# rbarile17/kelpie

Measured on AMD Instinct MI355X. Metric: candidate explanations evaluated/sec (incl. post-train) + rank-delta match rate, higher is better.
Workload: dtype bf16x3 (fp32-emulated)

## Files before the change

### kelpie_amd/csrc/kp_attn3.hpp

```cpp
#pragma once
#include <type_traits>

#include "kp_attn.hpp"

#ifdef KP_ATTN3_STAMPS
#ifndef KP_DIAGNOSTIC_BUILD
#error "KP_ATTN3_STAMPS is a diagnostic build (make diag / tools/attn_micro.sh)"
#endif
__device__ unsigned long long g_attn3_stamps[8];
#define KP3_STAMP(v) v = __builtin_amdgcn_s_memtime()
#define KP3_ACC(i, a, b) st_acc[i] += (b) - (a)
#else
#define KP3_STAMP(v) (void)0
#define KP3_ACC(i, a, b) (void)0
#endif

#ifdef KP_ATTN3_CLOCK
#ifndef KP_DIAGNOSTIC_BUILD
#error "KP_ATTN3_CLOCK is a diagnostic build (tools/attn_micro.sh)"
#endif
__device__ unsigned long long g_attn3_clock[4096][4];
#endif

#ifndef KP_O_AHEAD
#define KP_O_AHEAD 1
#endif
#ifndef KP_S_AHEAD
#define KP_S_AHEAD 1
#endif
static_assert(KP_S_AHEAD >= 1 && KP_S_AHEAD <= 2, "KP_S_AHEAD: 1..2 (lgkmcnt holds at most 15)");
#if (defined(KP_DIAG_NO_S) || defined(KP_DIAG_NO_O) || defined(KP_ATTN_NODMA) || defined(KP_DIAG_DMA_LGKM0) || \
     defined(KP_DMA_SPREAD_ALL) || defined(KP_DIAG_S4) || defined(KP_DIAG_DMA_VM0) || defined(KP_DIAG_M0SAVE) || defined(KP_DIAG_NO_OSTORE) || defined(KP_DIAG_EARLY_EXIT) || defined(KP_DIAG_O_HALF) || defined(KP_DIAG_S_HALF) || defined(KP_DIAG_XTILE_W)) && \
    !defined(KP_DIAGNOSTIC_BUILD)
#error "kp_attn3 diagnostic define without KP_DIAGNOSTIC_BUILD (these builds compute wrong results: make diag)"
#endif
#ifndef KP_DMA_SPREAD
#define KP_DMA_SPREAD 1
#endif
#ifndef KP_DMA_SPREAD_BCE
#define KP_DMA_SPREAD_BCE 0
#endif
#ifndef KP_ILV
#define KP_ILV 1
#endif
#ifndef KP_DMA_GROUP
#define KP_DMA_GROUP 1
#endif
#ifndef KP_ATTN_PRIO
#define KP_ATTN_PRIO 0
#endif
#ifndef KP_ATTN_FULLTILE
#define KP_ATTN_FULLTILE 1
#endif
#ifndef KP_ATTN_FULLTILE_ALL
#define KP_ATTN_FULLTILE_ALL 0
#endif
#ifndef KP_CV_EXACT_BCE
#define KP_CV_EXACT_BCE 0
#endif
#ifndef KP_ASM_ALL
#define KP_ASM_ALL 0
#endif
#ifndef KP_ASM_MIN_DB
#define KP_ASM_MIN_DB 13
#endif
#ifndef KP_O_NT
#define KP_O_NT 0
#endif
#ifndef KP_O_SC1
#define KP_O_SC1 0
#endif
#ifndef KP_BUF_DMA
#define KP_BUF_DMA 1
#endif
#ifdef KP_DIAG_NO_O
#define KP_DIAG_O false
#else
#define KP_DIAG_O true
#endif
static_assert(KP_O_AHEAD >= 1 && KP_O_AHEAD <= 2, "KP_O_AHEAD: 1..2 (lgkmcnt holds at most 15)");

namespace kpattn {

constexpr float kPosInf = __builtin_huge_valf();

typedef __bf16 bf16x8 __attribute__((ext_vector_type(8)));
typedef __bf16 bf16x4 __attribute__((ext_vector_type(4)));
typedef short s16x4 __attribute__((ext_vector_type(4)));

__host__ __device__ constexpr int split3_row_bytes(int DP) { return 3 * 2 * DP + ((DP / 16) % 2 ? 0 : 32); }
__host__ __device__ constexpr int split3_tile_bytes(int DP) { return 32 * split3_row_bytes(DP); }
__host__ __device__ constexpr int split3_pieces(int DP) { return (split3_tile_bytes(DP) + 1023) / 1024; }
__host__ __device__ constexpr bool attn3_asm(int DB) { return DB >= KP_ASM_MIN_DB || KP_ASM_ALL; }
__host__ __device__ constexpr bool attn3_bufdma(int DB) { return attn3_asm(DB) && KP_ILV && KP_BUF_DMA; }
__host__ __device__ constexpr int attn3_buf_pieces(int DB) {
  return attn3_bufdma(DB) ? (split3_pieces(16 * DB) + 3) / 4 * 4 : split3_pieces(16 * DB);
}
constexpr size_t attn3_lds_bytes(int DB) { return 2u * 1024u * (size_t)attn3_buf_pieces(DB); }

__device__ __forceinline__ void split3(float x, __bf16& h, __bf16& m, __bf16& l) {
  h = (__bf16)x;
  const float r1 = __fsub_rn(x, (float)h);
  m = (__bf16)r1;
  const float r2 = __fsub_rn(r1, (float)m);
  l = (__bf16)r2;
}

typedef __bf16 bf16v4 __attribute__((__vector_size__(8)));
template <bool ASM>
__device__ __forceinline__ bf16x8 lds_rd_bf8(uint32_t addr, int off) {
  if constexpr (ASM) {
    bf16x8 v;
    asm volatile("ds_read_b128 %0, %1 offset:%2" : "=v"(v) : "v"(addr), "i"(off));
    return v;
  } else {
    return *reinterpret_cast<const __attribute__((address_space(3))) bf16x8*>((uintptr_t)(addr + off));
  }
}
template <bool ASM>
__device__ __forceinline__ bf16x4 lds_rd_bf4(uint32_t addr, int off) {
  if constexpr (ASM) {
    bf16x4 v;
    asm volatile("ds_read_b64 %0, %1 offset:%2" : "=v"(v) : "v"(addr), "i"(off));
    return v;
  } else {
    return *reinterpret_cast<const __attribute__((address_space(3))) bf16x4*>((uintptr_t)(addr + off));
  }
}
template <bool ASM>
__device__ __forceinline__ bf16x4 lds_rd_tr(uint32_t addr, int off) {
  if constexpr (ASM) {
    bf16x4 v;
    asm volatile("ds_read_b64_tr_b16 %0, %1 offset:%2" : "=v"(v) : "v"(addr), "i"(off));
    return v;
  } else {
    const bf16v4 v = __builtin_amdgcn_ds_read_tr16_b64_v4bf16(
        reinterpret_cast<__attribute__((address_space(3))) bf16v4*>((uintptr_t)(addr + off)));
    return __builtin_bit_cast(bf16x4, v);
  }
}
template <bool ASM>
__device__ __forceinline__ bf16x8 tied3(bf16x8 v) {
  if constexpr (ASM) asm volatile("" : "+v"(v));
  return v;
}
template <bool ASM>
__device__ __forceinline__ bf16x4 tied3(bf16x4 v) {
  if constexpr (ASM) asm volatile("" : "+v"(v));
  return v;
}
template <bool ASM, int N>
__device__ __forceinline__ void lgkm_wait3() {
  if constexpr (ASM) lgkm_wait<N>();
}

constexpr int kPA[6] = {2, 1, 0, 1, 0, 0};
constexpr int kPB[6] = {0, 1, 2, 0, 1, 0};

__device__ __forceinline__ f32x4 mfma3(const bf16x8 (&a)[3], const bf16x8 (&b)[3], f32x4 c) {
  c = __builtin_amdgcn_mfma_f32_16x16x32_bf16(a[2], b[0], c, 0, 0, 0);
  c = __builtin_amdgcn_mfma_f32_16x16x32_bf16(a[1], b[1], c, 0, 0, 0);
  c = __builtin_amdgcn_mfma_f32_16x16x32_bf16(a[0], b[2], c, 0, 0, 0);
  c = __builtin_amdgcn_mfma_f32_16x16x32_bf16(a[1], b[0], c, 0, 0, 0);
  c = __builtin_amdgcn_mfma_f32_16x16x32_bf16(a[0], b[1], c, 0, 0, 0);
  c = __builtin_amdgcn_mfma_f32_16x16x32_bf16(a[0], b[0], c, 0, 0, 0);
  return c;
}
__device__ __forceinline__ f32x4 mfma3_k16(const bf16x4 (&a)[3], const bf16x4 (&b)[3], f32x4 c) {
#define KP_M16(x, y) \
  c = __builtin_amdgcn_mfma_f32_16x16x16bf16_1k(__builtin_bit_cast(s16x4, x), __builtin_bit_cast(s16x4, y), c, 0, 0, 0)
  KP_M16(a[2], b[0]);
  KP_M16(a[1], b[1]);
  KP_M16(a[0], b[2]);
  KP_M16(a[1], b[0]);
  KP_M16(a[0], b[1]);
  KP_M16(a[0], b[0]);
#undef KP_M16
  return c;
}

template <int DP>
__global__ void kp_split3_table(const float* __restrict__ E, int n_ent, uint8_t* __restrict__ out) {
  const long long i = (long long)blockIdx.x * blockDim.x + threadIdx.x;
  if (i >= (long long)n_ent * (DP / 2)) return;
  const int e = (int)(i / (DP / 2)), d = 2 * (int)(i % (DP / 2));
  __bf16 h[2], m[2], l[2];
  split3(E[(size_t)e * DP + d], h[0], m[0], l[0]);
  split3(E[(size_t)e * DP + d + 1], h[1], m[1], l[1]);
  __bf16* row = reinterpret_cast<__bf16*>(out + (size_t)e * split3_row_bytes(DP));
  row[d] = h[0];
  row[d + 1] = h[1];
  row[DP + d] = m[0];
  row[DP + d + 1] = m[1];
  row[2 * DP + d] = l[0];
  row[2 * DP + d + 1] = l[1];
}

template <int DB, int MODE>
constexpr int attn3_min_wgs() { return (MODE == ATT_BCE_O && 2 * attn3_lds_bytes(DB) <= 163840) ? 2 : 1; }

template <int DB, int MODE>
__global__ __launch_bounds__(256, (attn3_min_wgs<DB, MODE>())) void kp_attn3(const uint8_t* __restrict__ E3, int n_ent,
                                                   const float* __restrict__ Qpre, int nq, AttnWork wk,
                                                   float* __restrict__ out_m, float* __restrict__ out_l,
                                                   float* __restrict__ out_O, const float* __restrict__ qscale,
                                                   float ylo, const double* __restrict__ colpre) {
  constexpr bool WITH_O = MODE != ATT_SOFTMAX;
  constexpr int DP = 16 * DB;
  constexpr bool ASM = attn3_asm(DB);
  constexpr bool ILV = ASM && KP_ILV;
  constexpr int NK = DP / 32;
  constexpr int TAIL = (DP % 32) / 16;
  constexpr int KT = 32;
  constexpr int PART_B = 2 * DP;
  constexpr int ROW_B = split3_row_bytes(DP);
  constexpr bool BUFDMA = attn3_bufdma(DB);
  constexpr int PIECES = attn3_buf_pieces(DB);
  constexpr int BUF_B = 1024 * PIECES;
  extern __shared__ __attribute__((aligned(16))) uint8_t lds3[];

  const int tid = threadIdx.x;
#ifdef KP_DIAG_EARLY_EXIT
  if (ylo != 12345.f) return;
#endif
  if constexpr (KP_ATTN_PRIO > 0) __builtin_amdgcn_s_setprio(KP_ATTN_PRIO);
  const int lane = tid & 63;
  const int w = __builtin_amdgcn_readfirstlane(tid >> 6);
  const int g = lane >> 4, c = lane & 15;
  int key_begin = 0, key_end = 0;
  const uint32_t lds0 = (uint32_t)(uintptr_t)(__attribute__((address_space(3))) uint8_t*)lds3;
#ifdef KP_ATTN3_STAMPS
  unsigned long long st0 = 0, st1 = 0, st2 = 0, st3 = 0, st4 = 0;
  unsigned long long st_acc[5] = {0, 0, 0, 0, 0};
#endif

  const __amdgpu_buffer_rsrc_t e3rsrc = __builtin_amdgcn_make_buffer_rsrc(
      const_cast<uint8_t*>(E3), (short)0, (int)((n_ent + 31) / 32 * 32 * ROW_B + 1024), 0x00020000);
#if KP_O_SC1
  const __amdgpu_buffer_rsrc_t orsrc =
      __builtin_amdgcn_make_buffer_rsrc(out_O, (short)0, 0x7FFFFFFF, 0x00020000);
#endif
  auto bdma = [&](int tile, int buf, int p) {
    __builtin_amdgcn_raw_ptr_buffer_load_lds(
        e3rsrc, (__attribute__((address_space(3))) void*)(uintptr_t)(lds0 + (uint32_t)(buf * BUF_B + 1024 * p)), 16,
        16 * lane, (key_begin + tile * KT) * ROW_B + 1024 * p, 0, 0);
  };
  typedef int i32x4_t __attribute__((ext_vector_type(4)));
  const i32x4_t e3rs = {(int)(uint32_t)(uintptr_t)E3,
                        (int)(uint32_t)((uintptr_t)E3 >> 32) & 0xFFFF,
                        (int)((n_ent + 31) / 32 * 32 * ROW_B + 1024), 0x00020000};
  auto dma_group = [&](int tile, int buf, int g) {
    const int pb = w * ((PIECES + 3) / 4) + 4 * g;
    const uint32_t m0v = (uint32_t)__builtin_amdgcn_readfirstlane((int)(lds0 + (uint32_t)(buf * BUF_B + 1024 * pb)));
    const uint32_t so = (uint32_t)__builtin_amdgcn_readfirstlane((key_begin + tile * KT) * ROW_B + 1024 * pb);
    const int nleft = (PIECES + 3) / 4 - 4 * g;
    uint32_t keep;
    if (nleft >= 4)
      asm volatile(
          "s_mov_b32 %0, m0\n\ts_nop 4\n\ts_mov_b32 m0, %1\n\ts_nop 0\n\t"
          "buffer_load_dwordx4 %2, %3, %4 offen lds\n\t"
          "buffer_load_dwordx4 %2, %3, %4 offen offset:1024 lds\n\t"
          "buffer_load_dwordx4 %2, %3, %4 offen offset:2048 lds\n\t"
          "buffer_load_dwordx4 %2, %3, %4 offen offset:3072 lds\n\ts_mov_b32 m0, %0" : "=&s"(keep) : "s"(m0v),
          "v"(16 * lane), "s"(e3rs), "s"(so)
          : "memory");
    else if (nleft == 3)
      asm volatile(
          "s_mov_b32 %0, m0\n\ts_nop 4\n\ts_mov_b32 m0, %1\n\ts_nop 0\n\t"
          "buffer_load_dwordx4 %2, %3, %4 offen lds\n\t"
          "buffer_load_dwordx4 %2, %3, %4 offen offset:1024 lds\n\t"
          "buffer_load_dwordx4 %2, %3, %4 offen offset:2048 lds\n\ts_mov_b32 m0, %0" : "=&s"(keep) : "s"(m0v),
          "v"(16 * lane), "s"(e3rs), "s"(so)
          : "memory");
    else if (nleft == 2)
      asm volatile(
          "s_mov_b32 %0, m0\n\ts_nop 4\n\ts_mov_b32 m0, %1\n\ts_nop 0\n\t"
          "buffer_load_dwordx4 %2, %3, %4 offen lds\n\t"
          "buffer_load_dwordx4 %2, %3, %4 offen offset:1024 lds\n\ts_mov_b32 m0, %0" : "=&s"(keep) : "s"(m0v),
          "v"(16 * lane), "s"(e3rs), "s"(so)
          : "memory");
    else if (nleft == 1)
      asm volatile(
          "s_mov_b32 %0, m0\n\ts_nop 4\n\ts_mov_b32 m0, %1\n\ts_nop 0\n\t"
          "buffer_load_dwordx4 %2, %3, %4 offen lds\n\ts_mov_b32 m0, %0" : "=&s"(keep) : "s"(m0v),
          "v"(16 * lane), "s"(e3rs), "s"(so)
          : "memory");
  };
  constexpr bool DGROUP = KP_DMA_GROUP && BUFDMA;
  auto issue = [&](int tile, int buf) {
    const uint8_t* src = E3 + (size_t)(key_begin + tile * KT) * ROW_B + 16 * lane;
    if constexpr (KP_DMA_GROUP && BUFDMA) {
#pragma unroll
      for (int g = 0; g < ((PIECES + 3) / 4 + 3) / 4; ++g) dma_group(tile, buf, g);
      return;
    }
#pragma unroll
    for (int p0 = 0; p0 < PIECES; p0 += 4) {
      const int p = p0 + w;
      if constexpr (BUFDMA)
        bdma(tile, buf, p);
      else if (p < PIECES)
        glds16<ASM>(reinterpret_cast<const float*>(src + 1024 * p),
               __builtin_amdgcn_readfirstlane(lds0 + (uint32_t)(buf * BUF_B + 1024 * p)));
    }
  };
  constexpr int NPW = (PIECES + 3) / 4;
  constexpr int SPM = MODE == ATT_BCE_O ? KP_DMA_SPREAD_BCE : KP_DMA_SPREAD;
#ifdef KP_DMA_SPREAD_ALL
  constexpr bool SPREAD = SPM && WITH_O && KP_DIAG_O;
#else
  constexpr bool SPREAD = SPM && ASM && WITH_O && KP_DIAG_O;
#endif
  constexpr int NSLOT = (DP / 32 + (DP % 32) / 16) + (SPM == 3 ? 0 : DB);
  constexpr bool SPREAD2 = SPREAD && ILV && SPM >= 2;
  auto issue_piece = [&](int tile, int buf, int k) {
    const int p = 4 * k + w;
    if constexpr (BUFDMA)
      bdma(tile, buf, p);
    else if (p < PIECES)
      glds16<ASM>(reinterpret_cast<const float*>(E3 + (size_t)(key_begin + tile * KT) * ROW_B + 16 * lane + 1024 * p),
             __builtin_amdgcn_readfirstlane(lds0 + (uint32_t)(buf * BUF_B + 1024 * p)));
  };
  auto dma_slot = [&](int tile, int buf, int slot) {
#pragma unroll
    for (int k = 0; k < NPW; ++k)
      if ((k * NSLOT) / NPW == slot) issue_piece(tile, buf, k);
  };
#ifdef KP_ATTN3_CLOCK
  unsigned long long ck_t0, ck_r0;
  asm volatile("s_memtime %0\n\ts_memrealtime %1\n\ts_waitcnt lgkmcnt(0)" : "=s"(ck_t0), "=s"(ck_r0)::"memory");
#endif
  const int QT = (nq + 63) / 64;
  const long long total = (long long)QT * wk.ktq;
  long long it = wk.ranges ? 0 : (long long)blockIdx.x * wk.per_wg;
  const long long it_end = wk.ranges ? 0 : min(total, it + (long long)wk.per_wg);
  const int n_units = QT * wk.ranges;
  int unit = ((int)gridDim.x % 8 == 0) ? (int)(blockIdx.x % 8) * (int)(gridDim.x / 8) + (int)(blockIdx.x / 8)
                                       : (int)blockIdx.x;
  for (;;) {
    int qt, kt0, kt1, part;
    bool fill_rest;
    if (wk.ranges) {
      if (unit >= n_units) break;
      qt = unit % QT;
      part = unit / QT;
      kt0 = (int)((long long)part * wk.ktq / wk.ranges);
      kt1 = (int)((long long)(part + 1) * wk.ktq / wk.ranges);
      fill_rest = false;
      unit += (int)gridDim.x;
    } else {
      if (it >= it_end) break;
      qt = (int)(it / wk.ktq);
      kt0 = (int)(it - (long long)qt * wk.ktq);
      kt1 = (int)min((long long)wk.ktq, (long long)kt0 + (it_end - it));
      part = (int)blockIdx.x - (int)(((long long)qt * wk.ktq) / wk.per_wg);
      fill_rest = kt1 == wk.ktq;
      it += kt1 - kt0;
    }
    key_begin = kt0 * KT;
    key_end = min(n_ent, kt1 * KT);
    const int ntiles = kt1 - kt0;
    const int q = qt * 64 + 16 * w + c;
    const bool valid = q < nq;
    bf16x8 qb[NK > 0 ? NK : 1][3];
    bf16x4 qt4[3];
    float gsc = 0.f;
    if (MODE == ATT_BCE_O) gsc = valid ? qscale[q] : 0.f;
    {
      const float* qp = Qpre + (size_t)(valid ? q : 0) * DP;
#pragma unroll
      for (int s = 0; s < NK; ++s) {
        const float4 v0 = *reinterpret_cast<const float4*>(qp + 32 * s + 8 * g);
        const float4 v1 = *reinterpret_cast<const float4*>(qp + 32 * s + 8 * g + 4);
        const float f[8] = {v0.x, v0.y, v0.z, v0.w, v1.x, v1.y, v1.z, v1.w};
#pragma unroll
        for (int j = 0; j < 8; ++j) {
          __bf16 h, m, l;
          split3(valid ? f[j] : 0.f, h, m, l);
          qb[s][0][j] = h;
          qb[s][1][j] = m;
          qb[s][2][j] = l;
        }
      }
      if (TAIL) {
        const float4 v0 = *reinterpret_cast<const float4*>(qp + 32 * NK + 4 * g);
        const float f[4] = {v0.x, v0.y, v0.z, v0.w};
#pragma unroll
        for (int j = 0; j < 4; ++j) {
          __bf16 h, m, l;
          split3(valid ? f[j] : 0.f, h, m, l);
          qt4[0][j] = h;
          qt4[1][j] = m;
          qt4[2][j] = l;
        }
      }
    }
    f32x4 O[WITH_O ? DB : 1];
    float m_ref = kNegInf, l_run = 0.f;
    float csh = 0.f;

    for (int pass = 0; pass < 2; ++pass) {
#pragma unroll
      for (int j = 0; j < (WITH_O ? DB : 1); ++j) O[j] = (f32x4){0.f, 0.f, 0.f, 0.f};
      l_run = 0.f;
      float m_seen = kNegInf;
      if (ntiles > 0) issue(0, 0);
      asm volatile("s_waitcnt vmcnt(0)" ::: "memory");
      __syncthreads();
#ifdef KP_DIAG_XTILE_W
      float scp[2][4] = {{0.f, 0.f, 0.f, 0.f}, {0.f, 0.f, 0.f, 0.f}};
      float pwn[8] = {0.f, 0.f, 0.f, 0.f, 0.f, 0.f, 0.f, 0.f};
      float lacc = 0.f;
      bf16x8 pbn[3];
      float dtmp[8], htmp[8];
      auto wpiece = [&](int q) {
        if (q < 24) {
          const int j = q / 3, st = q % 3;
          if (st == 0) {
            dtmp[j] = scp[j >> 2][j & 3] - m_ref;
            m_seen = fmaxf(m_seen, scp[j >> 2][j & 3]);
          } else if (st == 1) {
            pwn[j] = __expf(dtmp[j]);
          } else {
            pwn[j] = __fsub_rn(pwn[j], csh);
            lacc += pwn[j];
          }
        } else if (q < 48) {
          const int j = (q - 24) / 3, st = (q - 24) % 3;
          if (st == 0) {
            const __bf16 h = (__bf16)pwn[j];
            pbn[0][j] = h;
            htmp[j] = __fsub_rn(pwn[j], (float)h);
          } else if (st == 1) {
            const __bf16 m = (__bf16)htmp[j];
            pbn[1][j] = m;
            htmp[j] = __fsub_rn(htmp[j], (float)m);
          } else {
            pbn[2][j] = (__bf16)htmp[j];
          }
        }
      };
#endif

      for (int t = 0; t < ntiles; ++t) {
        const int k0 = key_begin + t * KT;
        KP3_STAMP(st0);
        const bool dma_on = BUFDMA || t + 1 < ntiles;
        const int tn = t + 1 < ntiles ? t + 1 : t;
        const uint32_t tb = lds0 + (uint32_t)((t & 1) * BUF_B);
#if !defined(KP_ATTN_NODMA) && defined(KP_DMA_EARLY)
        if (t + 1 < ntiles) issue(t + 1, (t + 1) & 1);
#endif
        f32x4 sc[2] = {(f32x4){0.f, 0.f, 0.f, 0.f}, (f32x4){0.f, 0.f, 0.f, 0.f}};
#ifdef KP_DIAG_S4
        f32x4 sc4[2] = {(f32x4){0.f, 0.f, 0.f, 0.f}, (f32x4){0.f, 0.f, 0.f, 0.f}};
#endif
        const uint32_t rb = tb + (uint32_t)(c * ROW_B + 16 * g);
        const uint32_t rbt = rb - 8u * g;
        constexpr uint32_t SUB_B = 16u * ROW_B;
        static_assert(SUB_B + 3 * PART_B + 64 * NK < 65536, "LDS read offsets exceed the 16-bit offset field");
        constexpr int SA = ILV ? 2 : KP_S_AHEAD;
        constexpr int LAST = NK + TAIL - 1;
        bf16x8 ra[SA + 1][2][3];
        bf16x4 rt[2][3];
        auto load_full = [&](int s, int b) {
#pragma unroll
          for (int u = 0; u < 2; ++u)
#pragma unroll
            for (int p = 0; p < 3; ++p) ra[b][u][p] = lds_rd_bf8<ASM>(rb, (int)(u * SUB_B) + p * PART_B + 64 * s);
        };
        auto load_tail = [&]() {
#pragma unroll
          for (int u = 0; u < 2; ++u)
#pragma unroll
            for (int p = 0; p < 3; ++p)
              rt[u][p] = lds_rd_bf4<ASM>(rbt, (int)(u * SUB_B) + p * PART_B + 64 * NK);
        };
        auto load_step = [&](int j) {
          if (j < NK)
            load_full(j, j % (SA + 1));
          else
            load_tail();
        };
#ifndef KP_DIAG_NO_S
        if constexpr (ILV) {
          load_step(0);
          if (LAST >= 1) load_step(1);
#pragma unroll
          for (int s = 0; s <= LAST; ++s) {
            if (s < LAST)
              lgkm_wait<6>();
            else
              lgkm_wait<0>();
            __builtin_amdgcn_sched_barrier(0);
#if !defined(KP_ATTN_NODMA)
            if (SPREAD2 && dma_on) {
              dma_slot(tn, (t + 1) & 1, s);
              __builtin_amdgcn_sched_barrier(0);
            }
#endif
            const int b = s % 3;
#pragma unroll
            for (int k = 0; k < 6; ++k) {
#pragma unroll
              for (int u = 0; u < 2; ++u) {
#ifdef KP_DIAG_S4
                f32x4& acc = (s & 1) ? sc4[u] : sc[u];
#else
                f32x4& acc = sc[u];
#endif
                if (s < NK)
                  acc = __builtin_amdgcn_mfma_f32_16x16x32_bf16(ra[b][u][kPA[k]], qb[s < NK ? s : 0][kPB[k]], acc, 0, 0,
                                                               0);
                else
                  acc = __builtin_amdgcn_mfma_f32_16x16x16bf16_1k(__builtin_bit_cast(s16x4, rt[u][kPA[k]]),
                                                                  __builtin_bit_cast(s16x4, qt4[kPB[k]]), acc, 0, 0, 0);
#ifdef KP_DIAG_S_HALF
                if (u == 0 && s + 2 <= LAST && (k & 1) == 0) {
#else
                if (u == 0 && s + 2 <= LAST) {
#endif
                  const int j = s + 2, uu = k & 1, pp = k >> 1;
                  if (j < NK)
                    ra[j % 3][uu][pp] = lds_rd_bf8<true>(rb, (int)(uu * SUB_B) + pp * PART_B + 64 * j);
                  else
                    rt[uu][pp] = lds_rd_bf4<true>(rbt, (int)(uu * SUB_B) + pp * PART_B + 64 * NK);
                }
#ifdef KP_DIAG_XTILE_W
                if (u == 1 && WITH_O) wpiece(6 * s + k);
#endif
                __builtin_amdgcn_sched_barrier(0);
              }
            }
          }
#ifdef KP_DIAG_S4
          sc[0] += sc4[0];
          sc[1] += sc4[1];
#endif
        } else {
#pragma unroll
        for (int j = 0; j < SA && j <= LAST; ++j) load_step(j);
#pragma unroll
        for (int s = 0; s < NK; ++s) {
          if (s + SA <= LAST) {
            load_step(s + SA);
            lgkm_wait3<ASM, 6 * SA>();
          } else if (LAST - s >= 2) {
            lgkm_wait3<ASM, 12>();
          } else if (LAST - s == 1) {
            lgkm_wait3<ASM, 6>();
          } else {
            lgkm_wait3<ASM, 0>();
          }
#pragma unroll
          for (int u = 0; u < 2; ++u) {
            bf16x8 a[3];
#pragma unroll
            for (int p = 0; p < 3; ++p) a[p] = tied3<ASM>(ra[s % (SA + 1)][u][p]);
            sc[u] = mfma3(a, qb[s], sc[u]);
          }
        }
        if (TAIL) {
          lgkm_wait3<ASM, 0>();
#pragma unroll
          for (int u = 0; u < 2; ++u) {
            bf16x4 a[3];
#pragma unroll
            for (int p = 0; p < 3; ++p) a[p] = tied3<ASM>(rt[u][p]);
            sc[u] = mfma3_k16(a, qt4, sc[u]);
          }
        }
        }
#endif
#if !defined(KP_ATTN_NODMA) && !defined(KP_DMA_EARLY)
        if (!SPREAD && t + 1 < ntiles) issue(t + 1, (t + 1) & 1);
#endif
        const uint32_t ob = tb + (uint32_t)((4 * g + (c >> 2)) * ROW_B + 8 * (c & 3));
        constexpr int OA = ILV ? 2 : KP_O_AHEAD;
        bf16x4 ol[OA + 1][3], oh[OA + 1][3];
        auto load_o = [&](int m, int b) {
#pragma unroll
          for (int p = 0; p < 3; ++p) {
            ol[b][p] = lds_rd_tr<ASM>(ob, p * PART_B + 32 * m);
            oh[b][p] = lds_rd_tr<ASM>(ob, 16 * ROW_B + p * PART_B + 32 * m);
          }
        };
        KP3_STAMP(st1);
        if (WITH_O && KP_DIAG_O) {
#pragma unroll
          for (int m = 0; m < OA && m < DB; ++m) load_o(m, m);
        }
        float pw[2][4];
        auto weights = [&](auto full_c) {
          constexpr bool FULL = decltype(full_c)::value;
          auto keep = [&](int u, int r) { return FULL || (k0 + 16 * u + 4 * g + r < key_end); };
        if (MODE == ATT_BCE_O) {
#pragma unroll
          for (int u = 0; u < 2; ++u)
#pragma unroll
            for (int r = 0; r < 4; ++r) {
#if KP_CV_EXACT_BCE & 1
              const float x0 = 1.0f / (1.0f + expf(-sc[u][r]));
#else
              const float x0 = __builtin_amdgcn_rcpf(1.0f + __expf(-sc[u][r]));
#endif
              const float w0 = (1.0f - x0) * x0;
#if KP_CV_EXACT_BCE & 2
              const float gw = w0 >= 1e-12f ? (x0 - ylo) * gsc
                                            : (((x0 - ylo) * __builtin_amdgcn_rcpf(1e-12f)) * gsc) * w0;
              pw[u][r] = keep(u, r) ? gw : 0.f;
#else
              pw[u][r] = keep(u, r) ? (((x0 - ylo) * __builtin_amdgcn_rcpf(fmaxf(w0, 1e-12f))) * gsc) * w0 : 0.f;
#endif
            }
        } else {
          float v[2][4];
          float tmax = kNegInf;
#pragma unroll
          for (int u = 0; u < 2; ++u)
#pragma unroll
            for (int r = 0; r < 4; ++r) {
              v[u][r] = keep(u, r) ? sc[u][r] : kNegInf;
              tmax = fmaxf(tmax, v[u][r]);
            }
          m_seen = fmaxf(m_seen, tmax);
          if (pass == 0 && t == 0) {
            float mq = fmaxf(tmax, __shfl_xor(tmax, 16, 64));
            m_ref = fmaxf(mq, __shfl_xor(mq, 32, 64));
          }
#pragma unroll
          for (int u = 0; u < 2; ++u)
#pragma unroll
            for (int r = 0; r < 4; ++r) pw[u][r] = __expf(v[u][r] - m_ref);
        }
        {
          if (t == 0) {
            float mn = kPosInf;
#pragma unroll
            for (int u = 0; u < 2; ++u)
#pragma unroll
              for (int r = 0; r < 4; ++r)
                if (keep(u, r)) mn = fminf(mn, pw[u][r]);
            mn = fminf(mn, __shfl_xor(mn, 16, 64));
            mn = fminf(mn, __shfl_xor(mn, 32, 64));
            csh = (mn < kPosInf) ? mn : 0.f;
          }
          float lt = 0.f;
#pragma unroll
          for (int u = 0; u < 2; ++u) {
#pragma unroll
            for (int r = 0; r < 4; ++r) pw[u][r] = keep(u, r) ? __fsub_rn(pw[u][r], csh) : 0.f;
            lt += (pw[u][0] + pw[u][1]) + (pw[u][2] + pw[u][3]);
          }
          l_run += lt;
        }
        };
#ifdef KP_DIAG_XTILE_W
        if (t == 0 || !ILV || !WITH_O)
#endif
        if (KP_ATTN_FULLTILE && (ASM || KP_ATTN_FULLTILE_ALL) && k0 + KT <= key_end)
          weights(std::true_type{});
        else
          weights(std::false_type{});
        if (WITH_O && KP_DIAG_O) {
          bf16x8 pb[3];
#ifdef KP_DIAG_XTILE_W
          if (ILV && t > 0) {
            pb[0] = pbn[0];
            pb[1] = pbn[1];
            pb[2] = pbn[2];
            l_run += lacc;
            lacc = 0.f;
          } else
#endif
#pragma unroll
          for (int j = 0; j < 8; ++j) {
            __bf16 h, m, l;
            split3(pw[j >> 2][j & 3], h, m, l);
            pb[0][j] = h;
            pb[1][j] = m;
            pb[2][j] = l;
          }
#ifdef KP_DIAG_XTILE_W
#pragma unroll
          for (int u = 0; u < 2; ++u)
#pragma unroll
            for (int r = 0; r < 4; ++r) scp[u][r] = sc[u][r];
#endif
          KP3_STAMP(st2);
#pragma unroll
          for (int m = 0; m < DB; ++m) {
#if !defined(KP_ATTN_NODMA) && !defined(KP_DMA_EARLY)
            if (DGROUP && SPREAD && !SPREAD2 && dma_on) {
              if (m % 4 == 0 && m < NPW) dma_group(tn, (t + 1) & 1, m / 4);
              if (m == DB - 1)
                for (int g = (DB + 3) / 4; 4 * g < NPW; ++g) dma_group(tn, (t + 1) & 1, g);
            } else if (SPREAD && !SPREAD2 && dma_on) {
              if (m < NPW) {
                issue_piece(tn, (t + 1) & 1, m);
#ifdef KP_DIAG_DMA_LGKM0
                asm volatile("s_waitcnt lgkmcnt(0)" ::: "memory");
#endif
#ifdef KP_DIAG_DMA_VM0
                asm volatile("s_waitcnt vmcnt(0)" ::: "memory");
#endif
              }
              if (m == DB - 1)
                for (int k = DB; k < NPW; ++k) issue_piece(tn, (t + 1) & 1, k);
            }
#endif
            if constexpr (ILV) {
              if (m + 1 < DB)
                lgkm_wait<6>();
              else
                lgkm_wait<0>();
              __builtin_amdgcn_sched_barrier(0);
#if !defined(KP_ATTN_NODMA)
              if (SPREAD2 && dma_on) {
                dma_slot(tn, (t + 1) & 1, NK + TAIL + m);
                __builtin_amdgcn_sched_barrier(0);
              }
#endif
              bf16x8 a[3];
#pragma unroll
              for (int p = 0; p < 3; ++p) {
                const bf16x4 x = ol[m % 3][p], y = oh[m % 3][p];
                a[p] = (bf16x8){x[0], x[1], x[2], x[3], y[0], y[1], y[2], y[3]};
              }
#pragma unroll
              for (int k = 0; k < 6; ++k) {
                O[m] = __builtin_amdgcn_mfma_f32_16x16x32_bf16(a[kPA[k]], pb[kPB[k]], O[m], 0, 0, 0);
#ifdef KP_DIAG_O_HALF
                if (m + 2 < DB && ((m + 2) & 1) == 0) {
#else
                if (m + 2 < DB) {
#endif
                  const int mm = m + 2, pp = k >> 1;
                  if (k & 1)
                    oh[mm % 3][pp] = lds_rd_tr<true>(ob, 16 * ROW_B + pp * PART_B + 32 * mm);
                  else
                    ol[mm % 3][pp] = lds_rd_tr<true>(ob, pp * PART_B + 32 * mm);
                }
                __builtin_amdgcn_sched_barrier(0);
              }
              continue;
            }
            if (m + OA < DB) {
              load_o(m + OA, (m + OA) % (OA + 1));
              lgkm_wait3<ASM, 6 * OA>();
            } else if (DB - 1 - m >= 2) {
              lgkm_wait3<ASM, 12>();
            } else if (DB - 1 - m == 1) {
              lgkm_wait3<ASM, 6>();
            } else {
              lgkm_wait3<ASM, 0>();
            }
            bf16x8 a[3];
#pragma unroll
            for (int p = 0; p < 3; ++p) {
              const bf16x4 x = tied3<ASM>(ol[m % (OA + 1)][p]), y = tied3<ASM>(oh[m % (OA + 1)][p]);
              a[p] = (bf16x8){x[0], x[1], x[2], x[3], y[0], y[1], y[2], y[3]};
            }
            O[m] = mfma3(a, pb, O[m]);
          }
        }
        KP3_STAMP(st3);
        asm volatile("s_waitcnt vmcnt(0)" ::: "memory");
        __syncthreads();
        KP3_STAMP(st4);
        KP3_ACC(0, st0, st1);
        KP3_ACC(1, st1, st2);
        KP3_ACC(2, st2, st3);
        KP3_ACC(3, st3, st4);
#ifdef KP_ATTN3_STAMPS
        st_acc[4] += 1;
#endif
      }
      if (MODE == ATT_BCE_O) break;
      float mq = fmaxf(m_seen, __shfl_xor(m_seen, 16, 64));
      mq = fmaxf(mq, __shfl_xor(mq, 32, 64));
#if defined(KP_DIAG_NO_S) || defined(KP_DIAG_NO_O)
      break;
#endif
      if (pass == 1 || !__syncthreads_or(mq > m_ref + kMargin)) break;
      m_ref = mq;
    }

    float l_tot = l_run + __shfl_xor(l_run, 16, 64);
    l_tot += __shfl_xor(l_tot, 32, 64);
    if (ntiles > 0) {
      l_tot = __fmaf_rn(csh, (float)(key_end - key_begin), l_tot);
      if (WITH_O) {
        const double* p0 = colpre + (size_t)kt0 * DP;
        const double* p1 = colpre + (size_t)kt1 * DP;
#pragma unroll
        for (int m = 0; m < DB; ++m) {
          const int d = 16 * m + 4 * g;
          const double2 a0 = *reinterpret_cast<const double2*>(p0 + d), a1 = *reinterpret_cast<const double2*>(p0 + d + 2);
          const double2 b0 = *reinterpret_cast<const double2*>(p1 + d), b1 = *reinterpret_cast<const double2*>(p1 + d + 2);
          O[m][0] = __fmaf_rn(csh, (float)(b0.x - a0.x), O[m][0]);
          O[m][1] = __fmaf_rn(csh, (float)(b0.y - a0.y), O[m][1]);
          O[m][2] = __fmaf_rn(csh, (float)(b1.x - a1.x), O[m][2]);
          O[m][3] = __fmaf_rn(csh, (float)(b1.y - a1.y), O[m][3]);
        }
      }
    }
    if (valid) {
      const size_t o = (size_t)part * nq + q;
      if (g == 0 && MODE != ATT_BCE_O) {
        out_m[o] = m_ref;
        out_l[o] = l_tot;
      }
#ifdef KP_DIAG_NO_OSTORE
      if (false) {
#else
      if (WITH_O) {
#endif
        float* dst = out_O + o * DP;
#pragma unroll
        for (int m = 0; m < DB; ++m) {
#if KP_O_SC1
          typedef unsigned int u32x4_t __attribute__((ext_vector_type(4)));
          __builtin_amdgcn_raw_buffer_store_b128(__builtin_bit_cast(u32x4_t, O[m]), orsrc,
                                                 (int)((o * DP + 16 * m + 4 * g) * sizeof(float)), 0, 16);
#elif KP_O_NT
          __builtin_nontemporal_store(O[m], reinterpret_cast<f32x4*>(dst + 16 * m + 4 * g));
#else
          *reinterpret_cast<float4*>(dst + 16 * m + 4 * g) = make_float4(O[m][0], O[m][1], O[m][2], O[m][3]);
#endif
        }
      }
    }
    if (fill_rest && valid) {
      for (int pp = part + 1; pp < wk.n_parts; ++pp) {
        const size_t o = (size_t)pp * nq + q;
        if (g == 0 && MODE != ATT_BCE_O) {
          out_m[o] = kNegInf;
          out_l[o] = 0.f;
        }
        if (WITH_O) {
          float* dst = out_O + o * DP;
          for (int d = 4 * g; d < DP; d += 16) *reinterpret_cast<float4*>(dst + d) = make_float4(0.f, 0.f, 0.f, 0.f);
        }
      }
    }
  }
#ifdef KP_ATTN3_STAMPS
  if (lane == 0)
    for (int i = 0; i < 5; ++i) atomicAdd(&g_attn3_stamps[i], st_acc[i]);
#endif
#ifdef KP_ATTN3_CLOCK
  {
    unsigned long long ck_t1, ck_r1;
    asm volatile("s_waitcnt vmcnt(0)\n\ts_memtime %0\n\ts_memrealtime %1\n\ts_waitcnt lgkmcnt(0)"
                 : "=s"(ck_t1), "=s"(ck_r1)::"memory");
    if (tid == 0 && blockIdx.x < 4096) {
      g_attn3_clock[blockIdx.x][0] = ck_t0;
      g_attn3_clock[blockIdx.x][1] = ck_r0;
      g_attn3_clock[blockIdx.x][2] = ck_t1;
      g_attn3_clock[blockIdx.x][3] = ck_r1;
    }
  }
#endif
}

template <int DB>
const uint8_t* split3_image(kp_ctx* c) {
  constexpr int DP = 16 * DB;
  KP_REQUIRE(c->dp == DP, "attn3: table stride mismatch");
  if (!c->e3_ready) {
    const size_t n_pad = (size_t)(c->n_ent + 31) / 32 * 32;
    const size_t bytes = n_pad * split3_row_bytes(DP) + 1024;
    uint8_t* d = reinterpret_cast<uint8_t*>(c->e3.ensure(bytes));
    KP_HIP(hipMemsetAsync(d, 0, bytes, c->stream));
    const long long n = (long long)c->n_ent * (DP / 2);
    hipLaunchKernelGGL((kp_split3_table<DP>), dim3((unsigned)((n + 255) / 256)), dim3(256), 0, c->stream, c->dE,
                       c->n_ent, d);
    KP_HIP(hipGetLastError());
    c->e3_ready = true;
  }
  return c->e3.as<uint8_t>();
}

template <int DP>
__global__ void kp_tile_sums(const float* __restrict__ E, int n_ent, double* __restrict__ ts) {
  const int t = blockIdx.x, d = threadIdx.x;
  if (d >= DP) return;
  double s = 0.0;
  const int e1 = min(n_ent, 32 * t + 32);
  for (int e = 32 * t; e < e1; ++e) s += (double)E[(size_t)e * DP + d];
  ts[(size_t)t * DP + d] = s;
}
template <int DP>
__global__ void kp_tile_prefix(const double* __restrict__ ts, int ntiles, double* __restrict__ pre) {
  const int d = blockIdx.x * blockDim.x + threadIdx.x;
  if (d >= DP) return;
  double s = 0.0;
  pre[d] = 0.0;
  for (int t = 0; t < ntiles; ++t) {
    s += ts[(size_t)t * DP + d];
    pre[(size_t)(t + 1) * DP + d] = s;
  }
}
template <int DB>
const double* tile_prefix(kp_ctx* c) {
  constexpr int DP = 16 * DB;
  if (!c->e3pre_ready) {
    const int ntiles = (c->n_ent + 31) / 32;
    double* ts = reinterpret_cast<double*>(c->e3ts.ensure(sizeof(double) * (size_t)ntiles * DP));
    double* pre = reinterpret_cast<double*>(c->e3pre.ensure(sizeof(double) * (size_t)(ntiles + 1) * DP));
    hipLaunchKernelGGL((kp_tile_sums<DP>), dim3((unsigned)ntiles), dim3((DP + 63) / 64 * 64), 0, c->stream, c->dE,
                       c->n_ent, ts);
    KP_HIP(hipGetLastError());
    hipLaunchKernelGGL((kp_tile_prefix<DP>), dim3((DP + 63) / 64), dim3(64), 0, c->stream, ts, ntiles, pre);
    KP_HIP(hipGetLastError());
    c->e3pre_ready = true;
  }
  return c->e3pre.as<double>();
}

template <int DB, int MODE = ATT_SOFTMAX_O>
int attn3_wpc(kp_ctx* c) {
  static_assert(MODE == ATT_SOFTMAX_O || MODE == ATT_BCE_O, "attn3_wpc: the launched O mode");
  int& slot = c->attn3_wpc[MODE == ATT_BCE_O ? 1 : 0];
  if (slot <= 0) {
    int n = 0;
    KP_HIP(hipOccupancyMaxActiveBlocksPerMultiprocessor(&n, kp_attn3<DB, MODE>, 256, attn3_lds_bytes(DB)));
    slot = std::max(1, n);
  }
  return slot;
}

#define KP_DB_CASE(N, DB_MIN, ...)   \
  case N:                            \
    if constexpr (N >= (DB_MIN)) {   \
      constexpr int DB = N;          \
      __VA_ARGS__;                   \
    }                                \
    break;
#define KP_DB_DISPATCH(DBV, DB_MIN, MSG, ...)      \
  switch ((DBV) >= (DB_MIN) ? (DBV) : -1) {        \
    KP_DB_CASE(1, DB_MIN, __VA_ARGS__)             \
    KP_DB_CASE(2, DB_MIN, __VA_ARGS__)             \
    KP_DB_CASE(4, DB_MIN, __VA_ARGS__)             \
    KP_DB_CASE(8, DB_MIN, __VA_ARGS__)             \
    KP_DB_CASE(13, DB_MIN, __VA_ARGS__)            \
    KP_DB_CASE(16, DB_MIN, __VA_ARGS__)            \
    KP_DB_CASE(25, DB_MIN, __VA_ARGS__)            \
    default: throw KpError{KP_ENOTSUP, MSG};       \
  }

#ifndef KP_CV_ATTN_INFLIGHT
#define KP_CV_ATTN_INFLIGHT 0
#endif

inline AttnPlan attn_plan_ctx(const kp_ctx* c, int nq, int n_ent, int slots, bool inflight_ok) {
  if (c->attn_mode != 1) return attn_plan(nq, n_ent, slots);
  return attn_plan_select(c->attn_part, inflight_ok ? c->attn_inflight : 1, c->attn_ranges, nq, n_ent, slots);
}

inline void attn_plan_note(kp_ctx* c, const AttnPlan& p, int nq, bool inflight_ok) {
  if (nq < c->attn_last.nq) return;
  c->attn_last.nq = nq;
  c->attn_last.inflight = (c->attn_mode == 1 && inflight_ok) ? c->attn_inflight : 1;
  c->attn_last.ranges = p.wk.ranges;
  c->attn_last.n_parts = p.wk.n_parts;
  c->attn_last.n_wg = p.n_wg;
}

template <int DB, int MODE>
void launch_attn3(kp_ctx* c, int n_ent, const float* Q, int nq, const AttnPlan& plan, float* m, float* l, float* O,
                  const float* qscale, float ylo) {
  KP_REQUIRE(n_ent == c->n_ent, "attn3: key count differs from the table's (tile prefix sums)");
  KP_REQUIRE((long long)(n_ent + 31) / 32 * 32 * split3_row_bytes(16 * DB) + 1024 < (1LL << 31),
             "attn3: table too large for the 32-bit buffer descriptor of the split image");
  const uint8_t* E3 = split3_image<DB>(c);
  const double* pre = tile_prefix<DB>(c);
  hipLaunchKernelGGL((kp_attn3<DB, MODE>), dim3(plan.n_wg), dim3(256), attn3_lds_bytes(DB), c->stream, E3, n_ent, Q,
                     nq, plan.wk, m, l, O, qscale, ylo, pre);
  KP_HIP(hipGetLastError());
}

}
```

Measured before the change: 973.8.

## Add compile-time DMA slot placement table for attention tile prefetch

Introduces a constexpr slot-placement framework (kp_attn3_slots.hpp) that decides at which S or O MFMA step each prefetch DMA piece of the next key tile is issued. The kernel replaces the former spread/grouped DMA issue paths with a placed path driven by a preset (default equals KP_DMA_SPREAD), which can put loads into the S phase as well as the O phase. The aim is to interleave global-to-LDS loads more evenly with MFMA work so their latency is hidden. It adds template complexity, and DMA timing stamps for diagnostic builds.

```diff
diff --git a/kelpie_amd/csrc/kp_attn3.hpp b/kelpie_amd/csrc/kp_attn3.hpp
--- a/kelpie_amd/csrc/kp_attn3.hpp
+++ b/kelpie_amd/csrc/kp_attn3.hpp
@@ -1,7 +1,9 @@
 #pragma once
 #include <type_traits>
+#include <utility>
 
 #include "kp_attn.hpp"
+#include "kp_attn3_slots.hpp"
 
 #ifdef KP_ATTN3_STAMPS
 #ifndef KP_DIAGNOSTIC_BUILD
@@ -10,9 +12,25 @@
 __device__ unsigned long long g_attn3_stamps[8];
 #define KP3_STAMP(v) v = __builtin_amdgcn_s_memtime()
 #define KP3_ACC(i, a, b) st_acc[i] += (b) - (a)
+__device__ unsigned long long g_attn3_dma_stamps[4][3][2];
+#define KP_ATTN3_DMA_STAMPS 1
+#define KP3_DMA_T0()     \
+  int dma_here = 0;      \
+  const unsigned long long dt0 = __builtin_amdgcn_s_memtime()
+#define KP3_DMA_N(n) dma_here += (n)
+#define KP3_DMA_T1(slot)                                                         \
+  do {                                                                           \
+    const unsigned long long dt1 = __builtin_amdgcn_s_memtime();                 \
+    const int cls = (slot) < TL.ns ? 0 : (slot) < TL.first_o() ? 1 : 2;          \
+    dma_cyc[cls] += dma_here ? dt1 - dt0 : 0ull;                                 \
+    dma_n[cls] += (unsigned long long)dma_here;                                  \
+  } while (0)
 #else
 #define KP3_STAMP(v) (void)0
 #define KP3_ACC(i, a, b) (void)0
+#define KP3_DMA_T0() (void)0
+#define KP3_DMA_N(n) (void)0
+#define KP3_DMA_T1(slot) (void)0
 #endif
 
 #ifdef KP_ATTN3_CLOCK
@@ -36,6 +54,9 @@
 #endif
 #ifndef KP_DMA_SPREAD
 #define KP_DMA_SPREAD 1
+#endif
+#ifndef KP_DMA_PLACE
+#define KP_DMA_PLACE KP_DMA_SPREAD
 #endif
 #ifndef KP_DMA_SPREAD_BCE
 #define KP_DMA_SPREAD_BCE 0
@@ -148,6 +169,14 @@
 __device__ __forceinline__ bf16x4 tied3(bf16x4 v) {
   if constexpr (ASM) asm volatile("" : "+v"(v));
   return v;
+}
+template <int... I, class F>
+__device__ __forceinline__ void static_for_seq(std::integer_sequence<int, I...>, F&& f) {
+  (f(std::integral_constant<int, I>{}), ...);
+}
+template <int N, class F>
+__device__ __forceinline__ void static_for(F&& f) {
+  static_for_seq(std::make_integer_sequence<int, N>{}, f);
 }
 template <bool ASM, int N>
 __device__ __forceinline__ void lgkm_wait3() {
@@ -232,6 +261,7 @@
 #ifdef KP_ATTN3_STAMPS
   unsigned long long st0 = 0, st1 = 0, st2 = 0, st3 = 0, st4 = 0;
   unsigned long long st_acc[5] = {0, 0, 0, 0, 0};
+  unsigned long long dma_cyc[3] = {0, 0, 0}, dma_n[3] = {0, 0, 0};
 #endif
 
   const __amdgpu_buffer_rsrc_t e3rsrc = __builtin_amdgcn_make_buffer_rsrc(
@@ -286,6 +316,48 @@
           "v"(16 * lane), "s"(e3rs), "s"(so)
           : "memory");
   };
+#define KP3_DMA_ONE_WAVE(LOADS)                                                                        \
+  asm volatile("s_cmp_lg_u32 %5, %6\n\ts_cbranch_scc1 .Lkp3_dma_skip_%=\n\t"                            \
+               "s_mov_b32 %0, m0\n\ts_nop 4\n\ts_mov_b32 m0, %1\n\ts_nop 0\n\t" LOADS                  \
+               "s_mov_b32 m0, %0\n.Lkp3_dma_skip_%=:"                                                  \
+               : "=&s"(keep)                                                                           \
+               : "s"(m0v), "v"(16 * lane), "s"(e3rs), "s"(so), "s"(w), "i"(wv)                        \
+               : "memory", "scc")
+#define KP3_DMA_ALL_WAVES(LOADS)                                                               \
+  asm volatile("s_mov_b32 %0, m0\n\ts_nop 4\n\ts_mov_b32 m0, %1\n\ts_nop 0\n\t" LOADS "s_mov_b32 m0, %0" \
+               : "=&s"(keep)                                                                   \
+               : "s"(m0v), "v"(16 * lane), "s"(e3rs), "s"(so)                                  \
+               : "memory")
+#define KP3_DMA_RUN(LOADS)    \
+  do {                        \
+    if (wv < 0)               \
+      KP3_DMA_ALL_WAVES(LOADS); \
+    else                      \
+      KP3_DMA_ONE_WAVE(LOADS);  \
+  } while (0)
+  auto dma_run_wave = [&](int tile, int buf, int wv, int k0, int n) {
+    const int pb = (wv < 0 ? w : wv) * ((PIECES + 3) / 4) + k0;
+    const uint32_t m0v = (uint32_t)__builtin_amdgcn_readfirstlane((int)(lds0 + (uint32_t)(buf * BUF_B + 1024 * pb)));
+    const uint32_t so = (uint32_t)__builtin_amdgcn_readfirstlane((key_begin + tile * KT) * ROW_B + 1024 * pb);
+    uint32_t keep;
+    if (n >= 4)
+      KP3_DMA_RUN("buffer_load_dwordx4 %2, %3, %4 offen lds\n\t"
+                  "buffer_load_dwordx4 %2, %3, %4 offen offset:1024 lds\n\t"
+                  "buffer_load_dwordx4 %2, %3, %4 offen offset:2048 lds\n\t"
+                  "buffer_load_dwordx4 %2, %3, %4 offen offset:3072 lds\n\t");
+    else if (n == 3)
+      KP3_DMA_RUN("buffer_load_dwordx4 %2, %3, %4 offen lds\n\t"
+                  "buffer_load_dwordx4 %2, %3, %4 offen offset:1024 lds\n\t"
+                  "buffer_load_dwordx4 %2, %3, %4 offen offset:2048 lds\n\t");
+    else if (n == 2)
+      KP3_DMA_RUN("buffer_load_dwordx4 %2, %3, %4 offen lds\n\t"
+                  "buffer_load_dwordx4 %2, %3, %4 offen offset:1024 lds\n\t");
+    else if (n == 1)
+      KP3_DMA_RUN("buffer_load_dwordx4 %2, %3, %4 offen lds\n\t");
+  };
+#undef KP3_DMA_RUN
+#undef KP3_DMA_ALL_WAVES
+#undef KP3_DMA_ONE_WAVE
   constexpr bool DGROUP = KP_DMA_GROUP && BUFDMA;
   auto issue = [&](int tile, int buf) {
     const uint8_t* src = E3 + (size_t)(key_begin + tile * KT) * ROW_B + 16 * lane;
@@ -312,7 +384,8 @@
   constexpr bool SPREAD = SPM && ASM && WITH_O && KP_DIAG_O;
 #endif
   constexpr int NSLOT = (DP / 32 + (DP % 32) / 16) + (SPM == 3 ? 0 : DB);
-  constexpr bool SPREAD2 = SPREAD && ILV && SPM >= 2;
+  constexpr bool PLACED = SPREAD && ILV && KP_DMA_GROUP && BUFDMA && MODE != ATT_BCE_O;
+  constexpr bool SPREAD2 = SPREAD && ILV && SPM >= 2 && !PLACED;
   auto issue_piece = [&](int tile, int buf, int k) {
     const int p = 4 * k + w;
     if constexpr (BUFDMA)
@@ -325,6 +398,51 @@
 #pragma unroll
     for (int k = 0; k < NPW; ++k)
       if ((k * NSLOT) / NPW == slot) issue_piece(tile, buf, k);
+  };
+  static_assert(!PLACED || slots::preset_known(KP_DMA_PLACE), "KP_DMA_PLACE: a preset of kp_attn3_slots.hpp");
+  constexpr slots::Tile TL = slots::tile_of(DB);
+  constexpr int PL = KP_DMA_PLACE;
+  static_assert(!PLACED || (TL.npw == NPW && TL.ns == NK + TAIL && TL.nb == DB),
+                "kp_attn3_slots.hpp: the tile's slots and pieces differ from the kernel's");
+  static_assert(!PLACED || slots::preset_valid(PL, DB), "kp_attn3: the DMA placement breaks its invariants");
+  constexpr bool PL_S = PLACED && slots::uses_s(PL, TL);
+  constexpr bool PL_SKEW = PLACED && !slots::uniform(PL, TL);
+#ifndef KP_DIAGNOSTIC_BUILD
+  static_assert(!PL_SKEW, "kp_attn3: the wave-skewed placements are diagnostic builds (tools/attn_micro.sh)");
+#endif
+  auto dma_placed = [&](int tile, int buf, auto slot_c) __attribute__((always_inline)) {
+    constexpr int slot = decltype(slot_c)::value;
+    KP3_DMA_T0();
+    static_for<NPW>([&](auto k_c) __attribute__((always_inline)) {
+      constexpr int k = decltype(k_c)::value;
+      constexpr bool whole = k % 4 == 0 && slots::run_len(PL, TL, 0, k) == (NPW - k < 4 ? NPW - k : 4) &&
+                             slots::place(PL, TL, 0, k) == slot && slots::place(PL, TL, 1, k) == slot &&
+                             slots::place(PL, TL, 2, k) == slot && slots::place(PL, TL, 3, k) == slot;
+      if constexpr (whole) {
+        dma_group(tile, buf, k / 4);
+        KP3_DMA_N(slots::run_len(PL, TL, 0, k));
+      } else if constexpr (slots::uniform(PL, TL)) {
+        if constexpr (slots::place(PL, TL, 0, k) == slot && slots::run_len(PL, TL, 0, k) > 0) {
+          dma_run_wave(tile, buf, -1, k, slots::run_len(PL, TL, 0, k));
+          KP3_DMA_N(slots::run_len(PL, TL, 0, k));
+        }
+      } else {
+        static_for<slots::kWaves>([&](auto wv_c) __attribute__((always_inline)) {
+          constexpr int wv = decltype(wv_c)::value;
+          if constexpr (slots::place(PL, TL, wv, k) == slot && slots::run_len(PL, TL, wv, k) > 0) {
+            dma_run_wave(tile, buf, wv, k, slots::run_len(PL, TL, wv, k));
+            KP3_DMA_N(w == wv ? slots::run_len(PL, TL, wv, k) : 0);
+          }
+        });
+      }
+    });
+    KP3_DMA_T1(slot);
+  };
+  auto dma_at = [&](int tile, int buf, auto first_c, auto n_c, int i) __attribute__((always_inline)) {
+    static_for<decltype(n_c)::value>([&](auto j_c) __attribute__((always_inline)) {
+      if (decltype(j_c)::value == i)
+        dma_placed(tile, buf, std::integral_constant<int, decltype(first_c)::value + decltype(j_c)::value>{});
+    });
   };
 #ifdef KP_ATTN3_CLOCK
   unsigned long long ck_t0, ck_r0;
@@ -494,7 +612,12 @@
               lgkm_wait<0>();
             __builtin_amdgcn_sched_barrier(0);
 #if !defined(KP_ATTN_NODMA)
-            if (SPREAD2 && dma_on) {
+            if constexpr (PLACED) {
+              if constexpr (PL_S) {
+                dma_at(tn, (t + 1) & 1, std::integral_constant<int, 0>{}, std::integral_constant<int, NK + TAIL>{}, s);
+                __builtin_amdgcn_sched_barrier(0);
+              }
+            } else if (SPREAD2 && dma_on) {
               dma_slot(tn, (t + 1) & 1, s);
               __builtin_amdgcn_sched_barrier(0);
             }
@@ -691,7 +814,10 @@
 #pragma unroll
           for (int m = 0; m < DB; ++m) {
 #if !defined(KP_ATTN_NODMA) && !defined(KP_DMA_EARLY)
-            if (DGROUP && SPREAD && !SPREAD2 && dma_on) {
+            if constexpr (PLACED) {
+              if constexpr (!PL_SKEW)
+                dma_at(tn, (t + 1) & 1, std::integral_constant<int, TL.first_o()>{}, std::integral_constant<int, DB>{}, m);
+            } else if (DGROUP && SPREAD && !SPREAD2 && dma_on) {
               if (m % 4 == 0 && m < NPW) dma_group(tn, (t + 1) & 1, m / 4);
               if (m == DB - 1)
                 for (int g = (DB + 3) / 4; 4 * g < NPW; ++g) dma_group(tn, (t + 1) & 1, g);
@@ -715,6 +841,12 @@
               else
                 lgkm_wait<0>();
               __builtin_amdgcn_sched_barrier(0);
+#if !defined(KP_ATTN_NODMA) && !defined(KP_DMA_EARLY)
+              if constexpr (PL_SKEW) {
+                dma_at(tn, (t + 1) & 1, std::integral_constant<int, TL.first_o()>{}, std::integral_constant<int, DB>{}, m);
+                __builtin_amdgcn_sched_barrier(0);
+              }
+#endif
 #if !defined(KP_ATTN_NODMA)
               if (SPREAD2 && dma_on) {
                 dma_slot(tn, (t + 1) & 1, NK + TAIL + m);
@@ -846,8 +978,13 @@
     }
   }
 #ifdef KP_ATTN3_STAMPS
-  if (lane == 0)
+  if (lane == 0) {
     for (int i = 0; i < 5; ++i) atomicAdd(&g_attn3_stamps[i], st_acc[i]);
+    for (int i = 0; i < 3; ++i) {
+      atomicAdd(&g_attn3_dma_stamps[w][i][0], dma_cyc[i]);
+      atomicAdd(&g_attn3_dma_stamps[w][i][1], dma_n[i]);
+    }
+  }
 #endif
 #ifdef KP_ATTN3_CLOCK
   {
diff --git a/kelpie_amd/csrc/kp_attn3_slots.hpp b/kelpie_amd/csrc/kp_attn3_slots.hpp
--- /dev/null
+++ b/kelpie_amd/csrc/kp_attn3_slots.hpp
@@ -0,0 +1,146 @@
+#pragma once
+
+namespace kpattn {
+namespace slots {
+
+constexpr int kWaves = 4;
+constexpr int kMaxNpw = 32;
+constexpr int kRun = 4;
+constexpr int kMaxSlots = 64;
+
+struct Tile {
+  int ns, nw, nb, npw;
+  constexpr int n_slots() const { return ns + nw + nb; }
+  constexpr int first_o() const { return ns + nw; }
+};
+
+constexpr int tile_npw(int DB) {
+  const int DP = 16 * DB;
+  const int row = 3 * 2 * DP + ((DP / 16) % 2 ? 0 : 32);
+  const int pieces = (32 * row + 1023) / 1024;
+  return (pieces + 3) / 4;
+}
+constexpr Tile tile_of(int DB, int nw = 0) { return Tile{DB / 2 + DB % 2, nw, DB, tile_npw(DB)}; }
+
+enum Preset : int {
+  O_GROUPS = 1,
+  SO_EVEN = 2,
+  S_EVEN = 3,
+  SO_SINGLE_SKEW = 5,
+  SO_GROUPS_SKEW = 7,
+};
+constexpr int kPresets[] = {O_GROUPS, SO_EVEN, S_EVEN, SO_SINGLE_SKEW, SO_GROUPS_SKEW};
+constexpr int kNumPresets = sizeof(kPresets) / sizeof(kPresets[0]);
+constexpr bool preset_known(int p) {
+  for (int i = 0; i < kNumPresets; ++i)
+    if (kPresets[i] == p) return true;
+  return false;
+}
+
+constexpr int so_slot(Tile t, int j) { return j < t.ns ? j : t.nw + j; }
+
+constexpr int place(int preset, Tile t, int w, int k) {
+  const int g = k / kRun, ng = (t.npw + kRun - 1) / kRun;
+  switch (preset) {
+    case O_GROUPS:
+      return t.first_o() + (kRun * g < t.nb ? kRun * g : t.nb - 1);
+    case SO_EVEN:
+      return so_slot(t, k * (t.ns + t.nb) / t.npw);
+    case S_EVEN:
+      return k * t.ns / t.npw;
+    case SO_SINGLE_SKEW:
+      return so_slot(t, (kWaves * k + w) * (t.ns + t.nb) / (kWaves * t.npw));
+    case SO_GROUPS_SKEW:
+      return so_slot(t, (kWaves * g + w) * (t.ns + t.nb) / (kWaves * ng));
+    default:
+      return -1;
+  }
+}
+
+constexpr bool run_joins(int preset, Tile t, int w, int k) {
+  return k % kRun != 0 && k < t.npw && place(preset, t, w, k) == place(preset, t, w, k - 1);
+}
+constexpr int run_len(int preset, Tile t, int w, int k) {
+  if (k < 0 || k >= t.npw || run_joins(preset, t, w, k)) return 0;
+  int n = 1;
+  if (run_joins(preset, t, w, k + 1)) {
+    n = 2;
+    if (run_joins(preset, t, w, k + 2)) {
+      n = 3;
+      if (run_joins(preset, t, w, k + 3)) n = 4;
+    }
+  }
+  return n;
+}
+static_assert(kRun == 4, "run_len spells out runs of up to four pieces");
+constexpr bool uniform(int preset, Tile t) {
+  for (int w = 1; w < kWaves; ++w)
+    for (int k = 0; k < t.npw; ++k)
+      if (place(preset, t, w, k) != place(preset, t, 0, k)) return false;
+  return true;
+}
+constexpr bool uses_s(int preset, Tile t) {
+  for (int w = 0; w < kWaves; ++w)
+    for (int k = 0; k < t.npw; ++k)
+      if (place(preset, t, w, k) < t.ns) return true;
+  return false;
+}
+constexpr bool uses_window(int preset, Tile t) {
+  for (int w = 0; w < kWaves; ++w)
+    for (int k = 0; k < t.npw; ++k)
+      if (place(preset, t, w, k) >= t.ns && place(preset, t, w, k) < t.first_o()) return true;
+  return false;
+}
+
+struct Table {
+  Tile tile;
+  signed char slot[kWaves][kMaxNpw];
+  unsigned char run[kWaves][kMaxNpw];
+  unsigned char count[kWaves][kMaxSlots];
+  bool uniform;
+
+  constexpr Table(int preset, Tile t) : tile(t), slot{}, run{}, count{}, uniform(slots::uniform(preset, t)) {
+    for (int w = 0; w < kWaves; ++w) {
+      for (int k = 0; k < kMaxNpw; ++k) slot[w][k] = (signed char)(k < t.npw ? place(preset, t, w, k) : -1);
+      for (int k = 0; k < t.npw; ++k) run[w][k] = (unsigned char)run_len(preset, t, w, k);
+      for (int k = 0; k < t.npw; ++k) {
+        if (slot[w][k] >= 0 && slot[w][k] < kMaxSlots) ++count[w][slot[w][k]];
+      }
+    }
+  }
+
+  constexpr int pieces_at(int w, int s) const { return s >= 0 && s < kMaxSlots ? count[w][s] : 0; }
+
+  constexpr bool valid() const {
+    if (tile.npw < 1 || tile.npw > kMaxNpw || tile.n_slots() > kMaxSlots) return false;
+    for (int w = 0; w < kWaves; ++w) {
+      int seen[kMaxNpw] = {};
+      for (int s = 0; s < tile.n_slots(); ++s)
+        for (int k = 0; k < tile.npw; ++k)
+          if (slot[w][k] == s)
+            for (int j = 0; j < run[w][k]; ++j) {
+              if (k + j >= tile.npw || slot[w][k + j] != s) return false;
+              ++seen[k + j];
+            }
+      for (int k = 0; k < tile.npw; ++k) {
+        if (seen[k] != 1) return false;
+        if (slot[w][k] < 0 || slot[w][k] >= tile.n_slots()) return false;
+        if (k > 0 && slot[w][k] < slot[w][k - 1]) return false;
+        if (run[w][k] > kRun) return false;
+      }
+    }
+    return true;
+  }
+};
+
+constexpr bool preset_valid(int preset, int DB, int nw = 0) { return Table(preset, tile_of(DB, nw)).valid(); }
+constexpr bool all_presets_valid(int DB) {
+  for (int i = 0; i < kNumPresets; ++i)
+    if (!preset_valid(kPresets[i], DB)) return false;
+  return true;
+}
+static_assert(all_presets_valid(13) && all_presets_valid(16) && all_presets_valid(25),
+              "kp_attn3 DMA placement: a preset breaks the once-per-tile / inside-the-tile invariants");
+
+}
+}
```

Result: no change. 972.1 (median of 2 runs) (-0.2%).
